# GinZhu/RDST

Hardware: AMD Instinct MI355X
Metric: SR patches/sec fwd+bwd, RDST-E1 x4 64->256 (higher is better)
Workload: dtype bf16; 1 GPU; RDST-E1 x4 (RDST_E1_OASIS_example_SRx4.ini), 1x64x64 LR patches -> 256x256, step = fwd + L1 + bwd + flat-bucket grad all-reduce + Adam; global_batch=32, per_gpu_batch=32, parallelism=dp1, hip_graph=True, grad_bucket_bytes=17859844

## Files before the change

### rdst_amd/csrc/lnlin3_mfma.hip

```cpp
#include "linear.h"
#include "mfma.h"
#include "wattn_hd.h"
#include <stdlib.h>

#ifndef LB3_LOADW_SHAPE
#define LB3_LOADW_SHAPE(K, N) (((K) == 60 && (N) == 180) || ((K) == 90 && (N) == 270) || ((K) == 120 && (N) == 120))
#endif
#ifndef LB3_ABL
#define LB3_ABL 0
#endif

#ifdef LB3_STAMPS
#define LB3_T0 long long tk_[5] = {0, 0, 0, 0, 0}, tl_ = clock64();
#define LB3_T(i) { const long long n_ = clock64(); tk_[i] += n_ - tl_; tl_ = n_; }
#define LB3_TP(role) if (blockIdx.x == 0 && lane == 0) printf("wave %d %s: stash %lld  fetch %lld  barrier %lld  compute %lld  finish %lld\n", wave, role, tk_[0], tk_[1], tk_[2], tk_[3], tk_[4]);
#else
#define LB3_T0
#define LB3_T(i)
#define LB3_TP(role)
#endif

namespace {
using namespace wahd;
using MM = Mma<bf16>;

struct LB3Args {
  const bf16* X; int64_t ldx; const float* stats; const float* lnw; const float* W;
  const bf16* dY; int64_t lddy; bf16* dX; int64_t lddx; const bf16* Acc; int64_t ldacc;
  const bf16* Acc2; int64_t ldacc2;
  float* slab; int64_t slab_stride;
  int64_t M; int64_t ntiles; int tiles_per_wg;
};

__host__ __device__ constexpr int lb3_ldy(int NP) {
  const int b = NP * 2 + 16;
  return (b & 255) < 48 ? b + 64 : b;
}

template <int K_, int N_>
struct LB3 {
  static constexpr int K = K_, N = N_;
  static constexpr int NCT = (K + 1 + 31) / 32, NW = (N + 31) / 32, KN = (N + 15) / 16;
  static constexpr bool WIDE = N >= 180;
  static constexpr int TN = WIDE ? 3 : 1;
  static constexpr int TC = (K == 120 && N == 360) ? 2 : WIDE ? 1 : NCT;
  static_assert(NW % TN == 0 && NCT % TC == 0, "blocking");
  static constexpr int NGN = NW / TN, NGC = NCT / TC, NWG = NGN * NGC;
  static constexpr int NDG = NCT;
  static constexpr int NWV = NWG + NDG, NT = 64 * NWV;
  static constexpr int PKX = (K * 2 + 15) / 16, PKY = (N * 2 + 15) / 16;
  static constexpr int NY = 32 * PKY, NX = 32 * PKX;
  static constexpr bool LOADW = LB3_LOADW_SHAPE(K_, N_);
  static constexpr bool SPLITR = WIDE || LOADW;
  static constexpr int NTW = SPLITR ? 64 * NWG : NT, NTD = SPLITR ? 64 * NDG : NT;
  static constexpr int cdiv(int a, int b) { return (a + b - 1) / b; }
  static constexpr bool ACC_BY_W = K == 120 && N == 360;
  static constexpr int W_SY = cdiv(NY, NTW), W_SX = cdiv(NX, NTW), W_SA = (WIDE && !ACC_BY_W && !LOADW) ? 0 : cdiv(NX, NTW);
  static constexpr int D_SY = SPLITR ? 0 : W_SY, D_SX = SPLITR ? 0 : W_SX, D_SA = (ACC_BY_W || LOADW) ? 0 : cdiv(NX, NTD);
  static constexpr int CP = 32 * NCT;
  static constexpr int LDX = NCT == 4 ? 336 : CP * 2 + 16;
  static constexpr int LDY = lb3_ldy(32 * NW);
  static constexpr int OFF_AC = 32 * LDX, OFF_DY = 64 * LDX, OFF_SM = OFF_DY + 32 * LDY, BUF = OFF_SM + 128;
  static constexpr int OFF_RED = 2 * BUF;
  static constexpr int SMEM = OFF_RED + 2 * NCT * 256;
  static constexpr int PERCU0 = 12 / NWV < 1 ? 1 : 12 / NWV;
  static constexpr int PERCU1 = WIDE ? 1 : PERCU0 > 2 ? 2 : PERCU0;
  static constexpr int PERCU = PERCU1 * SMEM > 160 * 1024 ? 1 : PERCU1;
  static constexpr int WPS = (NWV * PERCU + 3) / 4;
};

template <class CF, bool LN, int SY, int SX, int SA>
struct LB3Loader {
  static constexpr int NS = SY + SX + SA;
  int meta[NS > 0 ? NS : 1];
  u32x4_a4 rd[NS > 0 ? NS : 1];
  u32x4_a4 rd2[SA > 0 ? SA : 1];
  float2 rst[SX > 0 ? SX : 1];
  static __device__ __forceinline__ int kind(int u) { return u < SY ? 0 : u < SY + SX ? 1 : 2; }
  __device__ __forceinline__ void setup(int tid_r, int ntr, bool has_acc) {
#pragma unroll
    for (int u = 0; u < NS; ++u) {
      const int kd = kind(u);
      const int idx = tid_r + ntr * (kd == 0 ? u : kd == 1 ? u - SY : u - SY - SX);
      const int per = kd == 0 ? CF::PKY : CF::PKX, rowbytes = kd == 0 ? CF::N * 2 : CF::K * 2;
      const bool on = idx < 32 * per && (kd != 2 || has_acc);
      const int row = on ? idx / per : 0, chk = on ? idx - row * per : 0;
      int o = chk * 16;
      if (o + 16 > rowbytes) o = rowbytes - 16;
      meta[u] = o | (row << 16) | ((on ? 1 : 0) << 24) | (((o & 15) == 0 ? 1 : 0) << 28);
    }
  }
  __device__ __forceinline__ void fetch(const LB3Args& p, int64_t tile) {
    const uint32_t Mu = (uint32_t)p.M;
#pragma unroll
    for (int u = 0; u < NS; ++u) {
      const int kd = kind(u);
      uint32_t row = (uint32_t)(tile * 32) + (uint32_t)((meta[u] >> 16) & 31);
      row = row < Mu ? row : Mu - 1;
      const char* base = reinterpret_cast<const char*>(kd == 0 ? p.dY : kd == 1 ? p.X : (p.Acc ? p.Acc : p.X));
      const uint32_t ldb = (uint32_t)((kd == 0 ? p.lddy : kd == 1 ? p.ldx : p.ldacc) * 2);
      rd[u] = *reinterpret_cast<const u32x4_a4*>(base + (size_t)(row * ldb + (uint32_t)(meta[u] & 0xffff)));
      if (kd == 2 && p.Acc2)
        rd2[u - SY - SX] = *reinterpret_cast<const u32x4_a4*>(reinterpret_cast<const char*>(p.Acc2) +
                                                              (size_t)(row * (uint32_t)(p.ldacc2 * 2) + (uint32_t)(meta[u] & 0xffff)));
      if (LN && kd == 1) rst[u - SY] = *reinterpret_cast<const float2*>(p.stats + 2 * (size_t)row);
    }
  }
  __device__ __forceinline__ void stash(const LB3Args& p, int64_t tile, char* buf) {
    const uint32_t Mu = (uint32_t)p.M;
#pragma unroll
    for (int u = 0; u < NS; ++u) {
      const int kd = kind(u);
      if (!((meta[u] >> 24) & 1)) continue;
      const int mrow = (meta[u] >> 16) & 31;
      const bool valid = (uint32_t)(tile * 32) + (uint32_t)mrow < Mu;
      Pack16 v;
      v.w[0] = valid ? rd[u].x : 0u; v.w[1] = valid ? rd[u].y : 0u; v.w[2] = valid ? rd[u].z : 0u; v.w[3] = valid ? rd[u].w : 0u;
      if (kd == 2 && p.Acc2) {
        const u32x4_a4 a = rd[u], b2 = rd2[u - SY - SX];
        const bool h1 = p.Acc != nullptr;
        float f[8];
        f[0] = bf16lo(b2.x) + (h1 ? bf16lo(a.x) : 0.f); f[1] = bf16hi(b2.x) + (h1 ? bf16hi(a.x) : 0.f);
        f[2] = bf16lo(b2.y) + (h1 ? bf16lo(a.y) : 0.f); f[3] = bf16hi(b2.y) + (h1 ? bf16hi(a.y) : 0.f);
        f[4] = bf16lo(b2.z) + (h1 ? bf16lo(a.z) : 0.f); f[5] = bf16hi(b2.z) + (h1 ? bf16hi(a.z) : 0.f);
        f[6] = bf16lo(b2.w) + (h1 ? bf16lo(a.w) : 0.f); f[7] = bf16hi(b2.w) + (h1 ? bf16hi(a.w) : 0.f);
#pragma unroll
        for (int e = 0; e < 8; ++e) f[e] = valid ? f[e] : 0.f;
        v = MM::pack(f);
      }
      if (LN && kd == 1) {
        const float2 st2 = rst[u - SY];
        float f[8];
        f[0] = bf16lo(rd[u].x); f[1] = bf16hi(rd[u].x); f[2] = bf16lo(rd[u].y); f[3] = bf16hi(rd[u].y);
        f[4] = bf16lo(rd[u].z); f[5] = bf16hi(rd[u].z); f[6] = bf16lo(rd[u].w); f[7] = bf16hi(rd[u].w);
#pragma unroll
        for (int e = 0; e < 8; ++e) f[e] = valid ? (f[e] - st2.x) * st2.y : 0.f;
        v = MM::pack(f);
        if ((meta[u] & 0xffff) == 0) reinterpret_cast<float*>(buf + CF::OFF_SM)[mrow] = st2.y;
      }
      int mt = meta[u];
      asm volatile("" : "+v"(mt));
      const int lrow = (mt >> 16) & 31, lo = mt & 0xffff;
      char* dst = buf + (kd == 0 ? CF::OFF_DY + lrow * CF::LDY : (kd == 2 ? CF::OFF_AC : 0) + lrow * CF::LDX) + lo;
      if ((meta[u] >> 28) & 1) *reinterpret_cast<Pack16*>(dst) = v;
      else {
        uint32_t* d = reinterpret_cast<uint32_t*>(dst);
        d[0] = v.w[0]; d[1] = v.w[1]; d[2] = v.w[2]; d[3] = v.w[3];
      }
    }
  }
};

template <int K, int N, bool LN>
__global__ void __launch_bounds__((LB3<K, N>::NT), (LB3<K, N>::WPS)) lnlin3_bwd_kernel(const LB3Args p) {
  extern __shared__ __attribute__((aligned(16))) char smem[];
  using CF = LB3<K, N>;
  constexpr int NCT = CF::NCT, NW = CF::NW, KN = CF::KN, TN = CF::TN, TC = CF::TC, NGC = CF::NGC, NWG = CF::NWG, NT = CF::NT;
  constexpr int LDX = CF::LDX, LDY = CF::LDY;
  const int tid = threadIdx.x, lane = tid & 63, wave = __builtin_amdgcn_readfirstlane(tid >> 6), r = lane & 31, hh = lane >> 5;
  const bool has_acc = p.Acc != nullptr || p.Acc2 != nullptr;

  if (!(LB3_ABL & 16)) lds_zero16(smem, CF::SMEM, tid, NT);
  __syncthreads();
  if (tid < 64) *reinterpret_cast<uint16_t*>(smem + (tid >> 5) * CF::BUF + (tid & 31) * LDX + K * 2) = 0x3f80;

  const int q = (lane & 15) >> 2, pp = lane & 3, gq1 = (lane >> 4) & 1;
  const int trc = (16 * gq1 + 4 * pp) * 2;
  const int tro_y = CF::OFF_DY + (8 * hh + q) * LDY + trc;
  const int tro_x = (8 * hh + q) * LDX + trc;

  const bool is_wg = wave < NWG;
  const int gn = wave / NGC, gc = wave - gn * NGC;
  const int dct = wave - NWG;

  const int64_t t0 = (int64_t)blockIdx.x * p.tiles_per_wg;
  const int64_t t1 = t0 + p.tiles_per_wg < p.ntiles ? t0 + p.tiles_per_wg : p.ntiles;
  __syncthreads();

  if (is_wg) {
    LB3Loader<CF, LN, CF::W_SY, CF::W_SX, CF::W_SA> ld;
    ld.setup(tid, CF::NTW, has_acc);
    if (t0 < t1) ld.fetch(p, t0);
    f32x16 G[TN][TC];
#pragma unroll
    for (int i = 0; i < TN; ++i)
#pragma unroll
      for (int j = 0; j < TC; ++j)
#pragma unroll
        for (int v = 0; v < 16; ++v) G[i][j][v] = 0.f;
    int b = 0;
    LB3_T0
    for (int64_t tile = t0; tile < t1; ++tile, b ^= 1) {
      char* buf = smem + b * CF::BUF;
      ld.stash(p, tile, buf);
      LB3_T(0)
      ld.fetch(p, tile + 1 < t1 ? tile + 1 : tile);
      LB3_T(1)
      __syncthreads();
      LB3_T(2)
#pragma unroll
      for (int s = 0; s < 2; ++s) {
        Pack16 ya[TN], xb[TC];
#pragma unroll
        for (int i = 0; i < TN; ++i) {
          const lds_cp yp = (lds_cp)(buf + tro_y + 16 * s * LDY) + (gn * TN + i) * 64;
          ya[i] = lds_tr_pack(yp, yp + 4 * LDY);
        }
#pragma unroll
        for (int j = 0; j < TC; ++j) {
          const lds_cp xp = (lds_cp)(buf + tro_x + 16 * s * LDX) + (gc * TC + j) * 64;
          xb[j] = lds_tr_pack(xp, xp + 4 * LDX);
        }
#pragma unroll
        for (int i = 0; i < TN; ++i)
#pragma unroll
          for (int j = 0; j < TC; ++j) {
#if !(LB3_ABL & 1)
            MM::mma(G[i][j], ya[i], xb[j]);
#else
            G[i][j][0] += __uint_as_float(ya[i].w[0] ^ xb[j].w[0]);
#endif
          }
      }
      LB3_T(3)
    }
    LB3_TP("wgrad")
    if (LN) __syncthreads();
    uint2* my = reinterpret_cast<uint2*>(p.slab) + (int64_t)blockIdx.x * p.slab_stride;
#pragma unroll
    for (int i = 0; i < TN; ++i)
#pragma unroll
      for (int j = 0; j < TC; ++j) {
        const int c = 32 * (gc * TC + j) + r;
#pragma unroll
        for (int g4 = 0; g4 < 4; ++g4) {
          const int n0 = 32 * (gn * TN + i) + 8 * g4 + 4 * hh;
          if (n0 < N && c <= K && !(LB3_ABL & 8))
            my[(int64_t)(n0 >> 2) * (K + 1) + c] =
                make_uint2(pack_bf16x2(G[i][j][4 * g4], G[i][j][4 * g4 + 1]), pack_bf16x2(G[i][j][4 * g4 + 2], G[i][j][4 * g4 + 3]));
        }
      }
    return;
  }

  LB3Loader<CF, LN, CF::D_SY, CF::D_SX, CF::D_SA> ld;
  ld.setup(CF::SPLITR ? tid - 64 * NWG : tid, CF::NTD, has_acc);
  if (t0 < t1) ld.fetch(p, t0);
  Pack16 wf[KN];
  {
    const int c = 32 * dct + r;
    const int cc = c < K ? c : K - 1;
    const float gm = (c < K) ? (LN ? p.lnw[cc] : 1.0f) : 0.f;
#pragma unroll
    for (int ks = 0; ks < KN; ++ks) {
      float f[8];
#pragma unroll
      for (int e = 0; e < 8; ++e) {
        const int n = 16 * ks + 8 * hh + e;
#if LB3_ABL & 4
        const float w = 0.01f * (float)(n + cc);
#else
        const float w = p.W[(size_t)(n < N ? n : N - 1) * K + cc];
#endif
        f[e] = n < N ? w * gm : 0.f;
      }
      wf[ks] = MM::pack(f);
    }
  }
  constexpr float invK = 1.0f / (float)K;
  float* red = reinterpret_cast<float*>(smem + CF::OFF_RED);
  f32x16 dx;
  u32x2_t xs[4], as[4];
  float rstd = 0.f;
  int64_t prow = -1;
  auto finish = [&](int pb) {
    float s1 = 0.f, s2 = 0.f;
    if (LN) {
#pragma unroll
      for (int w = 0; w < NCT; ++w) {
        const float2 v = *reinterpret_cast<const float2*>(red + ((pb * NCT + w) * 32 + r) * 2);
        s1 += v.x; s2 += v.y;
      }
      s1 *= invK; s2 *= invK;
    }
    float o[16];
#pragma unroll
    for (int g4 = 0; g4 < 4; ++g4) {
      const float xh[4] = {bf16lo(xs[g4].x), bf16hi(xs[g4].x), bf16lo(xs[g4].y), bf16hi(xs[g4].y)};
      const float ac[4] = {bf16lo(as[g4].x), bf16hi(as[g4].x), bf16lo(as[g4].y), bf16hi(as[g4].y)};
#pragma unroll
      for (int e = 0; e < 4; ++e) o[4 * g4 + e] = LN ? fmaf(rstd, dx[4 * g4 + e] - s1 - xh[e] * s2, ac[e]) : dx[4 * g4 + e] + ac[e];
    }
    if (prow < p.M) {
      bf16* drow = p.dX + prow * p.lddx;
#pragma unroll
      for (int gp2 = 0; gp2 < 2; ++gp2) {
        float c8[8];
#pragma unroll
        for (int e = 0; e < 4; ++e) {
          const auto sw = __builtin_amdgcn_permlane32_swap(__float_as_uint(o[8 * gp2 + e]), __float_as_uint(o[8 * gp2 + 4 + e]), false, false);
          c8[e] = __uint_as_float(sw[0]);
          c8[4 + e] = __uint_as_float(sw[1]);
        }
        const int cb = 32 * dct + 8 * (2 * gp2 + hh);
        if (cb + 8 <= K) {
          u32x4_a4 u;
          u.x = pack_bf16x2(c8[0], c8[1]); u.y = pack_bf16x2(c8[2], c8[3]);
          u.z = pack_bf16x2(c8[4], c8[5]); u.w = pack_bf16x2(c8[6], c8[7]);
          *reinterpret_cast<u32x4_a4*>(drow + cb) = u;
        } else {
#pragma unroll
          for (int e = 0; e < 8; ++e)
            if (cb + e < K) drow[cb + e] = __float2bfloat16(c8[e]);
        }
      }
    }
  };
  int b = 0;
  LB3_T0
  for (int64_t tile = t0; tile < t1; ++tile, b ^= 1) {
    char* buf = smem + b * CF::BUF;
    ld.stash(p, tile, buf);
    LB3_T(0)
    ld.fetch(p, tile + 1 < t1 ? tile + 1 : tile);
    LB3_T(1)
    __syncthreads();
    LB3_T(2)
    if (LN && prow >= 0) finish(b ^ 1);
    LB3_T(4)
    const lds_cp yrow = (lds_cp)(buf + CF::OFF_DY + r * LDY + hh * 16);
#pragma unroll
    for (int v = 0; v < 16; ++v) dx[v] = 0.f;
    if constexpr (KN > 12) {
#pragma unroll
      for (int ks = 0; ks < KN; ++ks) {
#if !(LB3_ABL & 2)
        MM::mma(dx, wf[ks], lds_pack(yrow + 32 * ks));
#else
        dx[0] += __uint_as_float(lds_pack(yrow + 32 * ks).w[0]);
#endif
      }
    } else {
      f32x16 d2;
#pragma unroll
      for (int v = 0; v < 16; ++v) d2[v] = 0.f;
#pragma unroll
      for (int ks = 0; ks < KN; ++ks) {
        const Pack16 yb = lds_pack(yrow + 32 * ks);
        if (ks & 1) MM::mma(d2, wf[ks], yb);
        else MM::mma(dx, wf[ks], yb);
      }
#pragma unroll
      for (int v = 0; v < 16; ++v) dx[v] += d2[v];
    }
    const lds_cp xrow = (lds_cp)(buf + r * LDX) + (32 * dct + 4 * hh) * 2;
#pragma unroll
    for (int g4 = 0; g4 < 4; ++g4) {
      xs[g4] = *reinterpret_cast<const LDS_AS u32x2_t*>(xrow + 16 * g4);
      as[g4] = *reinterpret_cast<const LDS_AS u32x2_t*>(xrow + CF::OFF_AC + 16 * g4);
    }
    prow = tile * 32 + r;
    if (LN) {
      rstd = reinterpret_cast<const float*>(buf + CF::OFF_SM)[r];
      float s1 = 0.f, s2 = 0.f;
#pragma unroll
      for (int g4 = 0; g4 < 4; ++g4) {
        const float xh[4] = {bf16lo(xs[g4].x), bf16hi(xs[g4].x), bf16lo(xs[g4].y), bf16hi(xs[g4].y)};
#pragma unroll
        for (int e = 0; e < 4; ++e) {
          s1 += dx[4 * g4 + e];
          s2 = fmaf(dx[4 * g4 + e], xh[e], s2);
        }
      }
      s1 = half_swap_sum(s1);
      s2 = half_swap_sum(s2);
      if (hh == 0) *reinterpret_cast<float2*>(red + ((b * NCT + dct) * 32 + r) * 2) = make_float2(s1, s2);
    } else {
      LB3_T(3)
      finish(b);
      LB3_T(4)
    }
    LB3_T(3)
  }
  LB3_TP("dgrad")
  if (LN) {
    __syncthreads();
    if (prow >= 0) finish(b ^ 1);
  }
}

template <int K, int N, bool LN>
int lb3_launch(LB3Args& p, int64_t max_wgs, int* grid_out, hipStream_t st) {
  using CF = LB3<K, N>;
  auto kern = lnlin3_bwd_kernel<K, N, LN>;
  static int percu_env = -1;
  if (percu_env < 0) { const char* e = rdst_dbg_getenv("RDST_LB3_PERCU"); percu_env = e ? atoi(e) : 0; }
  int per_cu = CF::PERCU;
  if (percu_env > 0 && percu_env < per_cu) per_cu = percu_env;
  int64_t cap = 256 * (int64_t)per_cu;
  if (cap > max_wgs) cap = max_wgs;
  int64_t grid = p.ntiles < cap ? p.ntiles : cap;
  p.tiles_per_wg = (int)((p.ntiles + grid - 1) / grid);
  grid = (p.ntiles + p.tiles_per_wg - 1) / p.tiles_per_wg;
  if (CF::SMEM > 64 * 1024) (void)hipFuncSetAttribute((const void*)kern, hipFuncAttributeMaxDynamicSharedMemorySize, CF::SMEM);
  hipLaunchKernelGGL(kern, dim3((unsigned)grid), dim3(CF::NT), CF::SMEM, st, p);
  *grid_out = (int)grid;
  return rdst_launch_status("lnlin3_bwd");
}

}

int lnlin3_bwd_bf16(const bf16* X, int64_t ldx, const float* ln_w, const float* stats, const float* Wt, const bf16* dY,
                    int64_t lddy, bf16* dX, int64_t lddx, const bf16* acc, int64_t ldacc, const bf16* acc2, int64_t ldacc2,
                    float* slab, int64_t slab_stride, int64_t M, int K, int N, int64_t max_wgs, int* grid_out, hipStream_t st) {
  static int off = -1;
  if (off < 0) { const char* e = rdst_dbg_getenv("RDST_LB3_OFF"); off = e ? atoi(e) : 0; }
  if (off) return RDST_ENOTSUP;
  const bool ln = ln_w != nullptr;
  LB3Args p{};
  p.X = X; p.ldx = ldx; p.stats = stats; p.lnw = ln_w; p.W = Wt; p.dY = dY; p.lddy = lddy; p.dX = dX; p.lddx = lddx;
  p.Acc = acc; p.ldacc = ldacc; p.Acc2 = acc2; p.ldacc2 = ldacc2; p.slab = slab; p.slab_stride = slab_stride; p.M = M;
  p.ntiles = (M + 31) / 32;
#define RDST_LB3(KK, NN, LL) if (K == KK && N == NN && ln == LL) return lb3_launch<KK, NN, LL>(p, max_wgs, grid_out, st);
  RDST_LB3(60, 180, true) RDST_LB3(90, 270, true) RDST_LB3(120, 360, true)
  RDST_LB3(60, 30, true) RDST_LB3(90, 30, true) RDST_LB3(120, 30, true)
  RDST_LB3(60, 60, false) RDST_LB3(90, 90, false) RDST_LB3(120, 120, false)
#undef RDST_LB3
  return RDST_ENOTSUP;
}
```

Measured before the change: 1990 patches/s.

## Stream LN-linear backward tiles via buffer-load-to-LDS three-slot ring

Adds a RING variant of the fused LayerNorm+linear backward kernel. It uses buffer_load_dwordx4 with the lds modifier to DMA X, Acc, Acc2, dY and stats tiles straight into a three-slot LDS ring, issuing two tiles ahead and waiting with vmcnt. An in-LDS pass then normalises X, writes the bias column, zero-pads dY and merges Acc2. This replaces the old register-staged load/stash double buffer and aims to hide global-load latency and free registers. It is enabled by default for shapes with N==K or K==60 when pointers are dword-aligned. It relies on buffer range checks for out-of-bounds rows and on m0 manipulation in inline asm.

Result: no change. 2000 patches/s, median of 6 (+0.5%).

```diff
diff --git a/rdst_amd/csrc/lnlin3_mfma.hip b/rdst_amd/csrc/lnlin3_mfma.hip
--- a/rdst_amd/csrc/lnlin3_mfma.hip
+++ b/rdst_amd/csrc/lnlin3_mfma.hip
@@ -2,6 +2,7 @@
 #include "mfma.h"
 #include "wattn_hd.h"
 #include <stdlib.h>
+#include <type_traits>
 
 #ifndef LB3_LOADW_SHAPE
 #define LB3_LOADW_SHAPE(K, N) (((K) == 60 && (N) == 180) || ((K) == 90 && (N) == 270) || ((K) == 120 && (N) == 120))
@@ -30,6 +31,7 @@
   const bf16* Acc2; int64_t ldacc2;
   float* slab; int64_t slab_stride;
   int64_t M; int64_t ntiles; int tiles_per_wg;
+  uint32_t nb_x, nb_dy, nb_acc, nb_acc2, nb_st;
 };
 
 __host__ __device__ constexpr int lb3_ldy(int NP) {
@@ -67,6 +69,20 @@
   static constexpr int PERCU1 = WIDE ? 1 : PERCU0 > 2 ? 2 : PERCU0;
   static constexpr int PERCU = PERCU1 * SMEM > 160 * 1024 ? 1 : PERCU1;
   static constexpr int WPS = (NWV * PERCU + 3) / 4;
+  static constexpr bool RING_OK = N == K || K == 60;
+  static constexpr bool A2OK = WIDE;
+  static constexpr int R_LDA = (K == 120 && N == 360) ? K * 2 : LDX;
+  static constexpr int R_OFF_AC = 32 * LDX, R_OFF_DY = R_OFF_AC + 32 * R_LDA, R_OFF_ST = R_OFF_DY + 32 * LDY;
+  static constexpr int R_OFF_A2 = R_OFF_ST + 256, R_SLOT = R_OFF_A2 + (A2OK ? 32 * R_LDA : 0);
+  static constexpr int NR = 3;
+  static constexpr int R_OFF_RED = NR * R_SLOT, R_SMEM = R_OFF_RED + 2 * NCT * 256;
+  static constexpr int SXS = LDX / 16, SAS = R_LDA / 16, SYS = LDY / 16;
+  static constexpr int DXS = (K * 2 + 15) / 16, DYS = (N * 2 + 15) / 16;
+  static constexpr int PX = cdiv(32 * SXS, 64), PA = cdiv(32 * SAS, 64), PY = cdiv(32 * SYS, 64);
+  static constexpr int XS = K * 2 / 16 + 1;
+  static constexpr bool PASS_ALL = NWG == 1;
+  static_assert(LDX % 16 == 0 && LDY % 16 == 0 && R_LDA % 16 == 0, "ring rows are whole slots");
+  static_assert(PERCU * R_SMEM <= 160 * 1024, "the ring keeps the register path's workgroups per CU");
 };
 
 template <class CF, bool LN, int SY, int SX, int SA>
@@ -151,22 +167,25 @@
   }
 };
 
-template <int K, int N, bool LN>
+template <int K, int N, bool LN, bool RING>
 __global__ void __launch_bounds__((LB3<K, N>::NT), (LB3<K, N>::WPS)) lnlin3_bwd_kernel(const LB3Args p) {
   extern __shared__ __attribute__((aligned(16))) char smem[];
   using CF = LB3<K, N>;
   constexpr int NCT = CF::NCT, NW = CF::NW, KN = CF::KN, TN = CF::TN, TC = CF::TC, NGC = CF::NGC, NWG = CF::NWG, NT = CF::NT;
   constexpr int LDX = CF::LDX, LDY = CF::LDY;
+  constexpr int SLOT = RING ? CF::R_SLOT : CF::BUF, OFF_DY = RING ? CF::R_OFF_DY : CF::OFF_DY;
+  constexpr int OFF_AC = RING ? CF::R_OFF_AC : CF::OFF_AC, LDA = RING ? CF::R_LDA : LDX;
+  constexpr int OFF_RED = RING ? CF::R_OFF_RED : CF::OFF_RED, SMEM = RING ? CF::R_SMEM : CF::SMEM;
   const int tid = threadIdx.x, lane = tid & 63, wave = __builtin_amdgcn_readfirstlane(tid >> 6), r = lane & 31, hh = lane >> 5;
   const bool has_acc = p.Acc != nullptr || p.Acc2 != nullptr;
 
-  if (!(LB3_ABL & 16)) lds_zero16(smem, CF::SMEM, tid, NT);
+  if (!(LB3_ABL & 16)) lds_zero16(smem, SMEM, tid, NT);
   __syncthreads();
-  if (tid < 64) *reinterpret_cast<uint16_t*>(smem + (tid >> 5) * CF::BUF + (tid & 31) * LDX + K * 2) = 0x3f80;
+  if (!RING && tid < 64) *reinterpret_cast<uint16_t*>(smem + (tid >> 5) * CF::BUF + (tid & 31) * LDX + K * 2) = 0x3f80;
 
   const int q = (lane & 15) >> 2, pp = lane & 3, gq1 = (lane >> 4) & 1;
   const int trc = (16 * gq1 + 4 * pp) * 2;
-  const int tro_y = CF::OFF_DY + (8 * hh + q) * LDY + trc;
+  const int tro_y = OFF_DY + (8 * hh + q) * LDY + trc;
   const int tro_x = (8 * hh + q) * LDX + trc;
 
   const bool is_wg = wave < NWG;
@@ -177,10 +196,121 @@
   const int64_t t1 = t0 + p.tiles_per_wg < p.ntiles ? t0 + p.tiles_per_wg : p.ntiles;
   __syncthreads();
 
+  typedef uint32_t u32x4s_t __attribute__((ext_vector_type(4)));
+  auto make_rsrc = [&](const void* ptr, uint32_t bytes) {
+    u32x4s_t rs;
+    rs.x = __builtin_amdgcn_readfirstlane((uint32_t)(uintptr_t)ptr);
+    rs.y = __builtin_amdgcn_readfirstlane((uint32_t)((uintptr_t)ptr >> 32) & 0xffffu);
+    rs.z = __builtin_amdgcn_readfirstlane(ptr ? bytes : 0u);
+    rs.w = 0x00020000u;
+    return rs;
+  };
+  const uint32_t lds0 = (uint32_t)(uintptr_t)(LDS_AS char*)smem;
+  constexpr int NPC = CF::PX + CF::PA + CF::PY + (LN ? 1 : 0) + (CF::A2OK ? CF::PA : 0);
+  constexpr int PCW = NPC / CF::NWG;
+  static_assert(PCW >= 1 && PCW < 64, "vmcnt is a 6-bit counter");
+  auto ring_issue = [&](int64_t tile, int slot) {
+    auto dma = [&](const u32x4s_t& rs, uint32_t ldst, uint32_t off) {
+      uint32_t keep;
+      asm volatile("s_mov_b32 %0, m0\n\ts_mov_b32 m0, %2\n\ts_nop 0\n\tbuffer_load_dwordx4 %1, %3, 0 offen lds\n\ts_mov_b32 m0, %0"
+                   : "=&s"(keep) : "v"(off), "s"(ldst), "s"(rs) : "memory");
+    };
+    const uint32_t tok0 = (uint32_t)(tile * 32), Mu = (uint32_t)p.M, sb = lds0 + (uint32_t)(slot * SLOT);
+    auto region = [&](auto S_, auto D_, auto P_, auto B_, const u32x4s_t& rs, uint32_t ldb, uint32_t off0) {
+      constexpr int S = decltype(S_)::value, D = decltype(D_)::value, P = decltype(P_)::value, B = decltype(B_)::value;
+      const int p0 = ((wave - B) % CF::NWG + CF::NWG) % CF::NWG;
+#pragma unroll
+      for (int k = 0; k < (P + CF::NWG - 1) / CF::NWG; ++k) {
+        const int pc = p0 + CF::NWG * k;
+        if (pc < P) {
+          const int qs = 64 * pc + lane, row = qs / S, cs = qs - row * S;
+          const uint32_t tr = tok0 + (uint32_t)row;
+          const uint32_t off = (cs < D && tr < Mu) ? tr * ldb + (uint32_t)(cs * 16) : 0xffffffffu;
+          if (qs < 32 * S) dma(rs, __builtin_amdgcn_readfirstlane(sb + (uint32_t)(off0 + 1024 * pc)), off);
+        }
+      }
+    };
+#define LB3_IC(v) std::integral_constant<int, (v)>()
+    region(LB3_IC(CF::SXS), LB3_IC(CF::DXS), LB3_IC(CF::PX), LB3_IC(0), make_rsrc(p.X, p.nb_x), (uint32_t)p.ldx * 2u, 0);
+    region(LB3_IC(CF::SAS), LB3_IC(CF::DXS), LB3_IC(CF::PA), LB3_IC(CF::PX), make_rsrc(p.Acc, p.nb_acc), (uint32_t)p.ldacc * 2u,
+           CF::R_OFF_AC);
+    region(LB3_IC(CF::SYS), LB3_IC(CF::DYS), LB3_IC(CF::PY), LB3_IC(CF::PX + CF::PA), make_rsrc(p.dY, p.nb_dy),
+           (uint32_t)p.lddy * 2u, CF::R_OFF_DY);
+    if constexpr (LN) {
+      if (((CF::PX + CF::PA + CF::PY) % CF::NWG) == wave) {
+        const uint32_t off = tok0 + (uint32_t)(2 * lane) < Mu ? tok0 * 8u + (uint32_t)(lane * 16) : 0xffffffffu;
+        if (lane < 16) dma(make_rsrc(p.stats, p.nb_st), __builtin_amdgcn_readfirstlane(sb + (uint32_t)CF::R_OFF_ST), off);
+      }
+    }
+    if constexpr (CF::A2OK)
+      region(LB3_IC(CF::SAS), LB3_IC(CF::DXS), LB3_IC(CF::PA), LB3_IC(CF::PX + CF::PA + CF::PY + (LN ? 1 : 0)),
+             make_rsrc(p.Acc2, p.nb_acc2), (uint32_t)p.ldacc2 * 2u, CF::R_OFF_A2);
+#undef LB3_IC
+  };
+  auto ring_pass = [&](int slot, int ptid, int ntp) {
+    char* sb = smem + slot * SLOT;
+    constexpr int XS = CF::XS, NXU = LN ? 32 * XS : 32;
+    for (int u = ptid; u < NXU; u += ntp) {
+      const int row = LN ? u / XS : u, cs = LN ? u - row * XS : XS - 1;
+      Pack16* dst = reinterpret_cast<Pack16*>(sb + row * LDX + cs * 16);
+      const Pack16 v = *dst;
+      Pack16 o;
+      if constexpr (LN) {
+        const float2 st2 = *reinterpret_cast<const float2*>(sb + CF::R_OFF_ST + row * 8);
+        float f[8];
+#pragma unroll
+        for (int e = 0; e < 4; ++e) {
+          f[2 * e] = bf16lo(v.w[e]);
+          f[2 * e + 1] = bf16hi(v.w[e]);
+        }
+#pragma unroll
+        for (int e = 0; e < 8; ++e) {
+          const int c = 8 * cs + e;
+          f[e] = c < K ? (f[e] - st2.x) * st2.y : (c == K ? 1.0f : 0.f);
+        }
+        o = MM::pack(f);
+      } else {
+#pragma unroll
+        for (int e = 0; e < 4; ++e) {
+          const int c = 8 * cs + 2 * e;
+          o.w[e] = c < K ? v.w[e] : (c == K ? 0x3f80u : 0u);
+        }
+      }
+      *dst = o;
+    }
+    if constexpr ((N * 2) % 16 != 0) {
+      for (int u = ptid; u < 32; u += ntp)
+#pragma unroll
+        for (int o = N * 2; o < CF::DYS * 16; o += 4) *reinterpret_cast<uint32_t*>(sb + OFF_DY + u * LDY + o) = 0u;
+    }
+    if constexpr (CF::A2OK) {
+      if (p.Acc2) {
+        const bool h1 = p.Acc != nullptr;
+        for (int u = ptid; u < 32 * CF::DXS; u += ntp) {
+          const int row = u / CF::DXS, cs = u - row * CF::DXS;
+          Pack16* dst = reinterpret_cast<Pack16*>(sb + OFF_AC + row * LDA + cs * 16);
+          const Pack16 a = *dst, b2 = *reinterpret_cast<const Pack16*>(sb + CF::R_OFF_A2 + row * LDA + cs * 16);
+          float f[8];
+#pragma unroll
+          for (int e = 0; e < 4; ++e) {
+            f[2 * e] = bf16lo(b2.w[e]) + (h1 ? bf16lo(a.w[e]) : 0.f);
+            f[2 * e + 1] = bf16hi(b2.w[e]) + (h1 ? bf16hi(a.w[e]) : 0.f);
+          }
+          *dst = MM::pack(f);
+        }
+      }
+    }
+  };
+
   if (is_wg) {
-    LB3Loader<CF, LN, CF::W_SY, CF::W_SX, CF::W_SA> ld;
-    ld.setup(tid, CF::NTW, has_acc);
-    if (t0 < t1) ld.fetch(p, t0);
+    LB3Loader<CF, LN, RING ? 0 : CF::W_SY, RING ? 0 : CF::W_SX, RING ? 0 : CF::W_SA> ld;
+    if constexpr (RING) {
+      ring_issue(t0, 0);
+      if (t0 + 1 < t1) ring_issue(t0 + 1, 1);
+    } else {
+      ld.setup(tid, CF::NTW, has_acc);
+      if (t0 < t1) ld.fetch(p, t0);
+    }
     f32x16 G[TN][TC];
 #pragma unroll
     for (int i = 0; i < TN; ++i)
@@ -188,16 +318,30 @@
       for (int j = 0; j < TC; ++j)
 #pragma unroll
         for (int v = 0; v < 16; ++v) G[i][j][v] = 0.f;
-    int b = 0;
+    int b = 0, rs = 0;
     LB3_T0
     for (int64_t tile = t0; tile < t1; ++tile, b ^= 1) {
-      char* buf = smem + b * CF::BUF;
+      char* buf = smem + (RING ? rs : b) * SLOT;
+      if constexpr (RING) {
+        if (tile + 1 < t1) asm volatile("s_waitcnt vmcnt(%0)" ::"n"(PCW) : "memory");
+        else asm volatile("s_waitcnt vmcnt(0)" ::: "memory");
+        LB3_T(1)
+        __syncthreads();
+        LB3_T(2)
+        if (tile + 2 < t1) ring_issue(tile + 2, rs == 0 ? 2 : rs - 1);
+        ring_pass(rs, tid, CF::PASS_ALL ? NT : 64 * NWG);
+        LB3_T(0)
+        __syncthreads();
+        LB3_T(2)
+        rs = rs == CF::NR - 1 ? 0 : rs + 1;
+      } else {
       ld.stash(p, tile, buf);
       LB3_T(0)
       ld.fetch(p, tile + 1 < t1 ? tile + 1 : tile);
       LB3_T(1)
       __syncthreads();
       LB3_T(2)
+      }
 #pragma unroll
       for (int s = 0; s < 2; ++s) {
         Pack16 ya[TN], xb[TC];
@@ -243,9 +387,11 @@
     return;
   }
 
-  LB3Loader<CF, LN, CF::D_SY, CF::D_SX, CF::D_SA> ld;
-  ld.setup(CF::SPLITR ? tid - 64 * NWG : tid, CF::NTD, has_acc);
-  if (t0 < t1) ld.fetch(p, t0);
+  LB3Loader<CF, LN, RING ? 0 : CF::D_SY, RING ? 0 : CF::D_SX, RING ? 0 : CF::D_SA> ld;
+  if constexpr (!RING) {
+    ld.setup(CF::SPLITR ? tid - 64 * NWG : tid, CF::NTD, has_acc);
+    if (t0 < t1) ld.fetch(p, t0);
+  }
   Pack16 wf[KN];
   {
     const int c = 32 * dct + r;
@@ -268,7 +414,7 @@
     }
   }
   constexpr float invK = 1.0f / (float)K;
-  float* red = reinterpret_cast<float*>(smem + CF::OFF_RED);
+  float* red = reinterpret_cast<float*>(smem + OFF_RED);
   f32x16 dx;
   u32x2_t xs[4], as[4];
   float rstd = 0.f;
@@ -316,10 +462,21 @@
       }
     }
   };
-  int b = 0;
+  int b = 0, rs = 0;
   LB3_T0
   for (int64_t tile = t0; tile < t1; ++tile, b ^= 1) {
-    char* buf = smem + b * CF::BUF;
+    char* buf = smem + (RING ? rs : b) * SLOT;
+    if constexpr (RING) {
+      __syncthreads();
+      LB3_T(2)
+      if (CF::PASS_ALL) ring_pass(rs, tid, NT);
+      LB3_T(0)
+      if (LN && prow >= 0) finish(b ^ 1);
+      LB3_T(4)
+      __syncthreads();
+      LB3_T(2)
+      rs = rs == CF::NR - 1 ? 0 : rs + 1;
+    } else {
     ld.stash(p, tile, buf);
     LB3_T(0)
     ld.fetch(p, tile + 1 < t1 ? tile + 1 : tile);
@@ -328,7 +485,8 @@
     LB3_T(2)
     if (LN && prow >= 0) finish(b ^ 1);
     LB3_T(4)
-    const lds_cp yrow = (lds_cp)(buf + CF::OFF_DY + r * LDY + hh * 16);
+    }
+    const lds_cp yrow = (lds_cp)(buf + OFF_DY + r * LDY + hh * 16);
 #pragma unroll
     for (int v = 0; v < 16; ++v) dx[v] = 0.f;
     if constexpr (KN > 12) {
@@ -354,14 +512,15 @@
       for (int v = 0; v < 16; ++v) dx[v] += d2[v];
     }
     const lds_cp xrow = (lds_cp)(buf + r * LDX) + (32 * dct + 4 * hh) * 2;
+    const lds_cp arow = (lds_cp)(buf + OFF_AC + r * LDA) + (32 * dct + 4 * hh) * 2;
 #pragma unroll
     for (int g4 = 0; g4 < 4; ++g4) {
       xs[g4] = *reinterpret_cast<const LDS_AS u32x2_t*>(xrow + 16 * g4);
-      as[g4] = *reinterpret_cast<const LDS_AS u32x2_t*>(xrow + CF::OFF_AC + 16 * g4);
+      as[g4] = *reinterpret_cast<const LDS_AS u32x2_t*>(arow + 16 * g4);
     }
     prow = tile * 32 + r;
     if (LN) {
-      rstd = reinterpret_cast<const float*>(buf + CF::OFF_SM)[r];
+      rstd = RING ? reinterpret_cast<const float*>(buf + CF::R_OFF_ST)[2 * r + 1] : reinterpret_cast<const float*>(buf + CF::OFF_SM)[r];
       float s1 = 0.f, s2 = 0.f;
 #pragma unroll
       for (int g4 = 0; g4 < 4; ++g4) {
@@ -389,10 +548,22 @@
   }
 }
 
+#ifndef LB3_RING
+#define LB3_RING 1
+#endif
+
 template <int K, int N, bool LN>
 int lb3_launch(LB3Args& p, int64_t max_wgs, int* grid_out, hipStream_t st) {
   using CF = LB3<K, N>;
-  auto kern = lnlin3_bwd_kernel<K, N, LN>;
+  auto dw = [](const void* q, int64_t ld) { return ((uintptr_t)q & 3) == 0 && (ld & 1) == 0; };
+  const bool ring = LB3_RING && CF::RING_OK && dw(p.X, p.ldx) && dw(p.dY, p.lddy) && (!p.Acc || dw(p.Acc, p.ldacc)) &&
+                    (!p.Acc2 || (CF::A2OK && dw(p.Acc2, p.ldacc2)));
+  auto kern = ring ? lnlin3_bwd_kernel<K, N, LN, true> : lnlin3_bwd_kernel<K, N, LN, false>;
+  const int smem = ring ? CF::R_SMEM : CF::SMEM;
+  auto span = [&](int64_t ld, int rowb) { return (uint32_t)((p.M - 1) * ld * 2 + rowb); };
+  p.nb_x = span(p.ldx, K * 2); p.nb_dy = span(p.lddy, N * 2);
+  p.nb_acc = p.Acc ? span(p.ldacc, K * 2) : 0; p.nb_acc2 = p.Acc2 ? span(p.ldacc2, K * 2) : 0;
+  p.nb_st = (uint32_t)(p.M * 8);
   static int percu_env = -1;
   if (percu_env < 0) { const char* e = rdst_dbg_getenv("RDST_LB3_PERCU"); percu_env = e ? atoi(e) : 0; }
   int per_cu = CF::PERCU;
@@ -402,8 +573,8 @@
   int64_t grid = p.ntiles < cap ? p.ntiles : cap;
   p.tiles_per_wg = (int)((p.ntiles + grid - 1) / grid);
   grid = (p.ntiles + p.tiles_per_wg - 1) / p.tiles_per_wg;
-  if (CF::SMEM > 64 * 1024) (void)hipFuncSetAttribute((const void*)kern, hipFuncAttributeMaxDynamicSharedMemorySize, CF::SMEM);
-  hipLaunchKernelGGL(kern, dim3((unsigned)grid), dim3(CF::NT), CF::SMEM, st, p);
+  if (smem > 64 * 1024) (void)hipFuncSetAttribute((const void*)kern, hipFuncAttributeMaxDynamicSharedMemorySize, smem);
+  hipLaunchKernelGGL(kern, dim3((unsigned)grid), dim3(CF::NT), smem, st, p);
   *grid_out = (int)grid;
   return rdst_launch_status("lnlin3_bwd");
 }
```
